# paulsengroup/modle

Hardware: AMD Instinct MI355X
Metric: simulated cells/sec (whole node), GRCh38 default barriers (higher is better)
Workload: dtype u32/f64

## Files before the change

modle_amd/csrc/sim_cell.h:

```cpp
#pragma once
#include "sim_rng.h"

namespace modle_dev {

struct Cell {
  const Params* p;
  const Interval* iv;
  Workspace ws;
  WaveLds lds;
  Rng g;
  u32 n_lefs;
  u32 n_active;
  u32 hist_len;
  u32 hist_head;
  u32 error;
  u32 n_hit[2];
  u32 n_rel;
  bool rel_valid;
  u32 n_bound;
  u32 n_keys;
  bool keys_valid;
  u32 n_disp[2];
  bool disp_valid;
  u32 max_fwd_move;
  bool inv_valid[2];
  bool filter_on;
  bool by_id_valid;
  u32 pair_seq;
  u32 pair_interval;
  bool pair_on;
  bool ring_lent;
#ifdef MODLE_PHASE_TIMERS
  u64 ph[16];
#endif
};
#if defined(MODLE_SUBTIMER_LEFBAR) || defined(MODLE_SUBTIMER_STATS) || defined(MODLE_SUBTIMER_RANK)
#define MODLE_SUBTIMER 1
#endif
#ifdef MODLE_SUBTIMER
#define MODLE_PH_ACTIVATION 1
#else
#define MODLE_PH_ACTIVATION 14
#endif
#ifdef MODLE_PHASE_TIMERS
#define PHASE(c, i, ...)                          \
  do {                                            \
    const u64 ph_t0_ = wave::clock();             \
    __VA_ARGS__;                                  \
    (c).ph[i] += wave::clock() - ph_t0_;          \
  } while (0)
#else
#define PHASE(c, i, ...) \
  do {                   \
    __VA_ARGS__;         \
  } while (0)
#endif
constexpr u32 REL_CAP = 2 * SORT_LDS_CAP;
constexpr u32 RANK_KEY_CAP = SORT_LDS_CAP - 1;
constexpr u32 RANK_KEY_CAP_BIG = RNG_RING - 1;
constexpr u32 RING_SPILL_AT = 64;
constexpr u32 ERR_LIST_OVERFLOW = 1;
constexpr u32 ERR_TRIAL_OVERFLOW = 2;
constexpr u32 ERR_INTERNAL = 3;
constexpr u32 ERR_MOVE_RANGE = 5;
constexpr bool NARROW_MOVES = sizeof(move_t) < sizeof(u32);

MODLE_DEV Interval interval_in_device_memory(const Interval& iv) {
  Interval g = iv;
  g.bar_pos = wave::as_global(iv.bar_pos);
  g.bar_dir = wave::as_global(iv.bar_dir);
  g.bar_stp_active = wave::as_global(iv.bar_stp_active);
  g.bar_stp_inactive = wave::as_global(iv.bar_stp_inactive);
  g.bar_occupancy = wave::as_global(iv.bar_occupancy);
  g.contacts = wave::as_global(iv.contacts);
  g.occupancy_1d = wave::as_global(iv.occupancy_1d);
  g.missed_updates = wave::as_global(iv.missed_updates);
  g.bar_bucket = wave::as_global(iv.bar_bucket);
  return g;
}

template <class T>
MODLE_DEV void swap_ptr(T*& a, T*& b) {
  T* t = a;
  a = b;
  b = t;
}

template <class T>
MODLE_DEV void swap_with_scratch(T*& a, u32*& scratch) {
  T* t = a;
  a = reinterpret_cast<T*>(scratch);
  scratch = reinterpret_cast<u32*>(t);
}
MODLE_DEV lefid_t* as_ids(u32* scratch) { return reinterpret_cast<lefid_t*>(scratch); }
MODLE_DEV const lefid_t* as_ids(const u32* scratch) { return reinterpret_cast<const lefid_t*>(scratch); }
MODLE_DEV move_t* as_moves(u32* scratch) { return reinterpret_cast<move_t*>(scratch); }
MODLE_DEV const move_t* as_moves(const u32* scratch) { return reinterpret_cast<const move_t*>(scratch); }

MODLE_DEV u32 bar_lower_bound(const Interval& iv, u64 key) {
  const u32 nb = iv.n_barriers;
  if (key <= iv.start) return 0;
  const u64 b = (key - iv.start) >> iv.bucket_shift;
  if (b >= iv.n_buckets) return nb;
  u32 i = iv.bar_bucket[b];
  while (i < nb && iv.bar_pos[i] < key) ++i;
  return i;
}

MODLE_DEV u32 lower_bound_u32(const u32* a, u32 n, u32 key) {
  u32 lo = 0, hi = n;
  while (lo < hi) {
    const u32 mid = (lo + hi) >> 1;
    if (a[mid] < key) lo = mid + 1; else hi = mid;
  }
  return lo;
}

template <bool FWD>
MODLE_DEV_NOINLINE void ensure_inverse(Cell& c) {
  if (c.inv_valid[FWD ? 1 : 0]) return;
  Workspace& ws = c.ws;
  const u32 n = wave::uniform(c.n_active);
  const u32 lane = wave::lane();
  const lefid_t* ids = FWD ? ws.f_id : ws.r_id;
  u32* rank = FWD ? ws.f_rank : ws.r_rank;
  const u32 nblk = (n + 255) / 256;
  for (u32 t = 0; t < nblk; ++t) {
    const u32 w = 256 * t + 4 * lane;
    const wave::U32x4 I = wave::ld4(ids, w < n ? w : 0u);
#pragma unroll
    for (u32 q = 0; q < 4; ++q) {
      if (w + q < n) rank[I.v[q]] = w + q;
    }
  }
  wave::sync_mem();
  c.inv_valid[FWD ? 1 : 0] = true;
}
MODLE_DEV void ensure_inverse_both(Cell& c) {
  ensure_inverse<false>(c);
  ensure_inverse<true>(c);
}

constexpr u32 RANK_HARD = 0x80000000u;
constexpr u32 RANK_FILTER_WORDS = SORT_LDS_CAP;
constexpr u32 RANK_FILTER_BITS = 64 * RANK_FILTER_WORDS;
MODLE_DEV void rank_filter_clear(Cell& c, u32 n_ids) {
  u64* bm = c.lds.sort_lds;
  const u32 nw = umin(RANK_FILTER_WORDS, (n_ids + 63) / 64);
  wave::lockstep();
  for (u32 k = wave::lane(); k < nw; k += 64) bm[k] = 0;
  wave::sync_lds();
}
MODLE_DEV void rank_filter_add_mask(Cell& c, u32 first, u64 members) {
  u64* bm = c.lds.sort_lds;
  if (wave::lane() == 0) bm[(first / 64) % RANK_FILTER_WORDS] |= members;
}
MODLE_DEV void rank_filter_add_id(Cell& c, u32 id) {
  u32* bm = reinterpret_cast<u32*>(c.lds.sort_lds);
  wave::lds_or_u32(&bm[(id % RANK_FILTER_BITS) >> 5], 1u << (id & 31u));
}
MODLE_DEV bool rank_filter_test(const Cell& c, u32 id) {
  const u32* bm = reinterpret_cast<const u32*>(c.lds.sort_lds);
  return ((bm[(id % RANK_FILTER_BITS) >> 5] >> (id & 31u)) & 1u) != 0;
}

}
```

modle_amd/csrc/sim_collisions.h:

```cpp
#pragma once

namespace modle_dev {

struct BoundaryCounts {
  u32 n5, n3;
};

MODLE_DEV_NOINLINE BoundaryCounts detect_boundaries(Cell& c) {
  Workspace& ws = c.ws;
  const u32 n = wave::uniform(c.n_active);
  const u32 lane = wave::lane();
  const u32 start = c.iv->start, last = c.iv->end - 1;
  const u32 first_fwd_pos = ws.f_pos[0];
  u32 last_rev_pos = 0;
  for (u32 top = n; top > 0;) {
    const u32 cnt = umin(64u, top);
    const bool act = lane < cnt;
    const u32 P = wave::ld_sel(ws.r_pos, top - 1 - lane, act, UNBOUND);
    const u64 m = wave::ballot(act && P != UNBOUND);
    if (m != 0) {
      last_rev_pos = wave::bcast(P, static_cast<u32>(wave::ctz64(m)));
      break;
    }
    top -= cnt;
// ... 805 lines not shown
        const u32 ps = wave_prefix_sum_u32(lane_cnt);
        const u32 first = n_listed + ps - lane_cnt;
#pragma unroll
        for (u32 j = 0; j < 4; ++j) {
          if (has[j]) {
            unit_rank[first + before[j]] = k[j];
            unit_entry[first + before[j]] = entry[j];
            unit_key[first + before[j]] = FWD ? hi_key[j] : lo_key[j];
          }
        }
        n_listed += wave::bcast(ps, 63);
      }
    }
  }
  wave::sync_mem();
  return n_listed;
}

template <bool FWD>
MODLE_DEV_NOINLINE void resolve_listed_units(Cell& c, u32 n_listed) {
  Workspace& ws = c.ws;
  const Params& p = *c.p;
  const u32 lane = wave::lane();
  const u32 nh = wave::uniform(c.n_hit[FWD ? 1 : 0]);
  const u32* hpos = ws.hit_pos[FWD ? 1 : 0];
  const u32* hidx = ws.hit_idx[FWD ? 1 : 0];
  const u32* unit_rank = ws.tmp[0];
  const u32* unit_entry = ws.tmp[1];
  const u32* unit_key = ws.tmp[2];
  u32* coll = FWD ? ws.f_coll : ws.r_coll;
  u32* barpos = stalling_barrier_positions<FWD>(ws);
  const f64 pb_major = wave::own_regs(p.pblock_major), pb_minor = wave::own_regs(p.pblock_minor);
  const bool major_trial = pb_major != 1.0, minor_trial = pb_minor != 1.0;
  const auto visit = [&](u32 e_lo, u32 e_hi, u32 q) { return FWD ? e_hi - 1 - q : e_lo + q; };
  for (u32 base = 0; base < n_listed; base += 64) {
    const u32 u = base + lane;
    const bool act = u < n_listed;
    const u32 k = wave::ld_sel(unit_rank, u, act, 0u);
    const u32 e0 = wave::ld_sel(unit_entry, u, act, 0u);
    const u32 key = wave::ld_sel(unit_key, u, act, 0u);
    u32 e_lo = e0, e_hi = e0;
    if (act) {
      if (!FWD) {
        while (e_lo > 0 && hpos[e_lo - 1] >= key) --e_lo;
      } else {
        while (e_hi < nh && hpos[e_hi] < key) ++e_hi;
      }
    }
    u32 ntr = 0;
    for (u32 q = 0; q < e_hi - e_lo; ++q) {
      const bool is_major = (hidx[visit(e_lo, e_hi, q)] & HITBAR_HARD) != 0;
      ntr += (is_major ? major_trial : minor_trial) ? 1u : 0u;
    }
    u32 off = wave_prefix_sum_u32(ntr);
    const u32 total = wave::bcast(off, 63);
    off -= ntr;
    const auto pick = [&](u32 first, u32& w_entry) {
      u32 t = 0;
      w_entry = 0xFFFFFFFFu;
      for (u32 q = 0; q < e_hi - e_lo; ++q) {
        const u32 e = visit(e_lo, e_hi, q);
        const bool is_major = (hidx[e] & HITBAR_HARD) != 0;
        bool hit = true;
        if (is_major ? major_trial : minor_trial) {
          hit = bernoulli_raw(rng_peek(c.g, c.g.pos + first + t), is_major ? pb_major : pb_minor);
          ++t;
        }
        if (hit) w_entry = e;
      }
    };
#ifdef MODLE_EMU_TRACE_RANK
    if (lane == 0) fprintf(stderr, "lef_bar_trials: %s batch of %u units, %u trials%s\n", FWD ? "fwd" : "rev",
                           umin(64u, n_listed - base), total, total > RNG_BLOCK ? " (resolved in rounds)" : "");
#endif
    u32 w_entry = 0xFFFFFFFFu;
    if (total <= RNG_BLOCK) {
      if (total != 0) rng_ensure(c.g, total);
      if (act) pick(off, w_entry);
      rng_advance(c.g, total);
    } else {
      u64 pend = wave::ballot(act);
      u32 base_tr = 0;
      while (pend != 0) {
        const bool mine_pending = ((pend >> lane) & 1u) != 0;
        const bool fits = mine_pending && (off + ntr - base_tr <= RNG_BLOCK);
        const u64 fm = wave::ballot(fits);
        if (fm == 0) {
          const u32 l = static_cast<u32>(wave::ctz64(pend));
          const u32 lo = wave::bcast(e_lo, l), hi = wave::bcast(e_hi, l);
          u32 w = 0xFFFFFFFFu;
          for (u32 q = 0; q < hi - lo; ++q) {
            const u32 e = FWD ? hi - 1 - q : lo + q;
            const bool is_major = (wave::uniform(hidx[e]) & HITBAR_HARD) != 0;
            bool hit = true;
            if (is_major ? major_trial : minor_trial) hit = bernoulli_raw(rng_next(c.g), is_major ? pb_major : pb_minor);
            if (hit) w = e;
          }
          if (lane == l) w_entry = w;
          base_tr += wave::bcast(ntr, l);
          pend &= ~(u64(1) << l);
        } else {
          const u32 l_last_fit = static_cast<u32>(63 - wave::clz64(fm));
          const u32 cnt = wave::bcast(off + ntr, l_last_fit) - base_tr;
          if (cnt != 0) rng_ensure(c.g, cnt);
          if (fits) pick(off - base_tr, w_entry);
          rng_advance(c.g, cnt);
          base_tr += cnt;
          pend &= ~fm;
        }
      }
    }
    if (w_entry != 0xFFFFFFFFu) {
      const u32 wd = hidx[w_entry];
      coll[k] = cw_make(wd & ~HITBAR_HARD, EV_COLLISION | EV_LEF_BAR) | ((wd & HITBAR_HARD) ? CW_HARD : 0u);
      barpos[k] = hpos[w_entry];
    }
  }
  wave::sync_mem();
}

template <bool FWD>
MODLE_DEV_NOINLINE void detect_lef_bar(Cell& c, BoundaryCounts bc) {
  if (wave::uniform(c.iv->n_barriers) == 0) return;
  if (!lef_bar_trials_needed(*c.p)) {
    detect_lef_bar_det<FWD>(c, bc);
    return;
  }
  const u32 n_listed = detect_lef_bar_sweep<FWD, true>(c, bc);
  if (n_listed != 0) resolve_listed_units<FWD>(c, n_listed);
}

MODLE_DEV void lef_lef_collision_pos(u32 rev_p, u32 fwd_p, u32 rev_move, u32 fwd_move,
                                     u32& out_rev, u32& out_fwd) {
  const f64 relative_speed = static_cast<f64>(rev_move) + static_cast<f64>(fwd_move);
  const f64 ttc = static_cast<f64>(rev_p - fwd_p) / relative_speed;
  const u32 cpos = fwd_p + static_cast<u32>(wave::f_round(static_cast<f64>(fwd_move) * ttc));
  if (cpos == fwd_p) {
    out_rev = cpos + 1;
    out_fwd = cpos;
  } else {
    out_rev = cpos;
    out_fwd = cpos - 1;
  }
}

MODLE_DEV u32 stalling_barrier_pos(const Interval& iv, u32 word) {
  const u32 idx = cw_index(word);
  return idx < iv.n_barriers ? iv.bar_pos[idx] : 0u;
}

#ifndef MODLE_PRIMARY_BACK
#define MODLE_PRIMARY_BACK 128
#endif
constexpr u32 PRIMARY_BACK = MODLE_PRIMARY_BACK;
static_assert(PRIMARY_BACK + 128 <= STAGE_CAP, "the slice must reach the block's last rank");
struct PrimaryBatch {
  wave::U32x2 R, rev_move;
  u32 sp[STAGE_CAP / 64];
};
template <class Op>
MODLE_DEV void primary_load_batch(Op op, const Workspace& ws, u32 n, u32 base, u32 w0, u32 lane,
                                  PrimaryBatch& b, bool rev_side) {
  if (rev_side) {
    const u32 k0 = base + 2 * lane;
    const u32 kq = k0 < n ? k0 : 0u;
    b.R = wave::ld2(ws.r_pos, kq);
    b.rev_move = wave::ld2(ws.r_move, kq);
  }
#pragma unroll
  for (u32 q = 0; q < STAGE_CAP / 64; ++q) {
    const u32 t = lane + 64 * q;
    b.sp[q] = op(ws.f_pos, w0 + t, w0 + t < n, UNBOUND, b.sp[q]);
  }
}

MODLE_DEV_NOINLINE void detect_primary(Cell& c, BoundaryCounts bc, bool fuse_correct) {
  Workspace& ws = c.ws;
  const Params& p = *c.p;
  const Interval& iv = *c.iv;
  const u32 n = wave::uniform(c.n_active);
  if (bc.n5 == n || bc.n3 == n) return;
  const u32 lane = wave::lane();
  const u32 i2 = bc.n3 == 0 ? n : n - (bc.n3 - 1);
  const f64 p_collide = 1.0 - p.p_bypass;
  const bool never_collide = p.p_bypass != 0.0 && p_collide == 0.0;
  const bool trials = p.p_bypass != 0.0 && !never_collide;
  const u32 prim = EV_COLLISION | EV_LEF_LEF_PRIMARY;
  u32* stage = c.lds.stage;
  u32* const q_k = ws.tmp[0];
  u32* const q_pf = ws.tmp[1];
  u32* const dump = reinterpret_cast<u32*>(ws.sort_keys) + 2 * lane;
  const u64 fwd_reach = wave::uniform(c.max_fwd_move);
  u32 n_cand = 0;
  u32 carry_pos = 0;
  const u32 first = bc.n5;
  const auto slice_start = [](u32 base) { return base > PRIMARY_BACK ? base - PRIMARY_BACK : 0u; };
  {
    const u32 b0 = first & ~1u;
    PrimaryBatch pa, pb;
    primary_load_batch(wave::LdRaw{}, ws, n, b0, slice_start(b0), lane, pa, true);
    if (b0 + 128 < n) primary_load_batch(wave::LdRaw{}, ws, n, b0 + 128, slice_start(b0 + 128), lane, pb, true);
    const auto block = [&](PrimaryBatch& cur, u32 base) {
      const u32 w0 = slice_start(base);
      primary_load_batch(wave::LdMask{}, ws, n, base, w0, lane, cur, false);
      u32 k[2], R[2], rev_move[2];
      bool act[2];
#pragma unroll
      for (u32 j = 0; j < 2; ++j) {
        k[j] = base + 2 * lane + j;
        act[j] = k[j] >= first && k[j] < n;
        R[j] = act[j] ? cur.R.v[j] : UNBOUND;
        rev_move[j] = act[j] ? cur.rev_move.v[j] : 0u;
      }
      wave::lockstep();
#pragma unroll
      for (u32 q = 0; q < STAGE_CAP / 64; ++q) stage[lane + 64 * q] = cur.sp[q];
      wave::sync_lds();
      if (base + 256 < n) primary_load_batch(wave::LdRaw{}, ws, n, base + 256, slice_start(base + 256), lane, cur, true);
      const u32 prev_in = wave::shfl_up1(R[1]);
      const u32 Rprev0 = lane > 0 ? prev_in : carry_pos;
      u32 lo[2] = {0, 0};
      static_assert(STAGE_CAP == 256, "the search below covers 256 entries");
#pragma unroll
      for (u32 sft = 128; sft >= 1; sft >>= 1) {
        u32 sv[2];
#pragma unroll
        for (u32 j = 0; j < 2; ++j) sv[j] = stage[lo[j] + sft - 1];
        wave::sched_fence();
#pragma unroll
        for (u32 j = 0; j < 2; ++j) {
          if (sv[j] < R[j]) lo[j] += sft;
        }
        wave::sched_fence();
      }
      const u32 st_last = stage[STAGE_CAP - 1];
      u32 pf[2] = {0, 0};
      bool beyond = false;
#pragma unroll
      for (u32 j = 0; j < 2; ++j) {
        u32 l = lo[j];
        if (l == STAGE_CAP - 1 && st_last < R[j]) l = STAGE_CAP;
        pf[j] = umin(w0 + l, n);
        beyond = beyond || (act[j] && ((l == 0 && w0 > 0) || (l == STAGE_CAP && w0 + STAGE_CAP < n)));
      }
      if (wave::any(beyond)) {
#pragma unroll
        for (u32 j = 0; j < 2; ++j) {
          const u32 l = pf[j] - w0;
          if (act[j] && ((l == 0 && w0 > 0) || (l == STAGE_CAP && w0 + STAGE_CAP < n)))
            pf[j] = lower_bound_u32(ws.f_pos, n, R[j]);
          wave::pin(pf[j]);
        }
      }
      u32 F[2];
      bool has[2], staged[2];
#pragma unroll
      for (u32 j = 0; j < 2; ++j) {
        has[j] = act[j] && pf[j] >= 1 && pf[j] < i2;
        const u32 kf = pf[j] - 1;
        staged[j] = has[j] && kf >= w0 && kf - w0 < STAGE_CAP;
        F[j] = stage[staged[j] ? kf - w0 : 0u];
      }
      wave::sched_fence();
      if (wave::any((has[0] && !staged[0]) || (has[1] && !staged[1]))) {
#pragma unroll
        for (u32 j = 0; j < 2; ++j) {
          if (has[j] && !staged[j]) F[j] = ws.f_pos[pf[j] - 1];
          wave::pin(F[j]);
        }
      }
      bool cand[2];
#pragma unroll
      for (u32 j = 0; j < 2; ++j) {
        const u32 Rprev = j == 0 ? Rprev0 : R[0];
        const bool first_after = (k[j] == first) || Rprev <= F[j];
        const u32 delta = R[j] - F[j];
        cand[j] = has[j] && first_after && static_cast<u64>(delta) < static_cast<u64>(rev_move[j]) + fwd_reach;
      }
      const u64 cm0 = wave::ballot(cand[0]), cm1 = wave::ballot(cand[1]);
      {
        const u64 lt = lanemask_lt(lane);
        const u32 e0 = n_cand + static_cast<u32>(wave::popc64(cm0 & lt) + wave::popc64(cm1 & lt));
        const u32 e1 = e0 + (cand[0] ? 1u : 0u);
        *(cand[0] ? &q_k[e0] : dump) = k[0];
        *(cand[0] ? &q_pf[e0] : dump + 1) = pf[0];
        *(cand[1] ? &q_k[e1] : dump) = k[1];
        *(cand[1] ? &q_pf[e1] : dump + 1) = pf[1];
      }
      n_cand += static_cast<u32>(wave::popc64(cm0) + wave::popc64(cm1));
      carry_pos = wave::bcast(R[1], 63);
    };
    for (u32 base = b0; base < n; base += 256) {
      block(pa, base);
      if (base + 128 < n) block(pb, base + 128);
    }
  }
  wave::sync_mem();
  struct PairRegs {
    u32 k, pf, R, rev_move, rev_id, rc, rbp, F, fwd_move, fwd_id, fc, fbp;
  };
  const auto load_pairs = [&](u32 base, u32 kk, u32 pp, PairRegs& r) {
    const bool in = base + lane < n_cand;
    const u32 k = in ? kk : 0u, kf = in ? pp - 1 : 0u;
    r.k = kk;
    r.pf = pp;
    r.R = wave::LdRaw{}(ws.r_pos, k, true, 0, 0u);
    r.rev_move = wave::LdRaw{}(ws.r_move, k, true, 0, 0u);
    r.rev_id = wave::LdRaw{}(ws.r_id, k, true, 0, 0u);
    r.rc = wave::LdRaw{}(ws.r_coll, k, true, 0, 0u);
    r.rbp = wave::LdRaw{}(stalling_barrier_positions<false>(ws), k, true, 0, 0u);
    r.F = wave::LdRaw{}(ws.f_pos, kf, true, 0, 0u);
    r.fwd_move = wave::LdRaw{}(ws.f_move, kf, true, 0, 0u);
    r.fwd_id = wave::LdRaw{}(ws.f_id, kf, true, 0, 0u);
    r.fc = wave::LdRaw{}(ws.f_coll, kf, true, 0, 0u);
    r.fbp = wave::LdRaw{}(stalling_barrier_positions<true>(ws), kf, true, 0, 0u);
  };
  const auto list_k = [&](u32 base) { return wave::ld_sel(q_k, base + lane, base + lane < n_cand, 0u); };
  const auto list_pf = [&](u32 base) { return wave::ld_sel(q_pf, base + lane, base + lane < n_cand, 1u); };
  PairRegs pcur;
  u32 nk = 0, np = 1;
  if (n_cand != 0) {
    load_pairs(0, list_k(0), list_pf(0), pcur);
    if (64 < n_cand) {
      nk = list_k(64);
      np = list_pf(64);
    }
  }
  for (u32 base = 0; base < n_cand; base += 64) {
    const PairRegs q = pcur;
    if (base + 64 < n_cand) {
      load_pairs(base + 64, nk, np, pcur);
      if (base + 128 < n_cand) {
        nk = list_k(base + 128);
        np = list_pf(base + 128);
      }
    }
    const bool valid = base + lane < n_cand;
    const u32 delta = q.R - q.F;
    const bool cand = valid && static_cast<u64>(delta) < static_cast<u64>(q.rev_move) + q.fwd_move;
    const u64 cm = wave::ballot(cand);
    bool hit = cand && !never_collide;
    if (trials && cm != 0) {
      const u32 cnt = static_cast<u32>(wave::popc64(cm));
      rng_ensure(c.g, cnt);
      const u32 t = static_cast<u32>(wave::popc64(cm & lanemask_lt(lane)));
      hit = cand && bernoulli_raw(rng_peek(c.g, c.g.pos + t), p_collide);
      rng_advance(c.g, cnt);
    }
    const auto handle_hit = [&](u32 pf_h, u32 k_h, u32 R_h, u32 F_h, u32 rev_move_h, u32 fwd_move_h, u32 rev_id_k_h,
                                u32 fwd_id_s_h, u32 rc_k_h, u32 fc_s_h, u32 rbp_k_h, u32 fbp_s_h) {
      const u32 kf = pf_h - 1;
      const u32 rev_id = rev_id_k_h, fwd_id = fwd_id_s_h;
      u32 cpos_rev, cpos_fwd;
      lef_lef_collision_pos(R_h, F_h, rev_move_h, fwd_move_h, cpos_rev, cpos_fwd);
      const u32 rc = rc_k_h, fc = fc_s_h;
      const bool rev_occ = cw_occurred(rc), fwd_occ = cw_occurred(fc);
      u32 rev_other = 0, fwd_other = 0;
      const bool rev_odd = rev_occ && !cw_occurred_as(rc, EV_LEF_BAR);
      const bool fwd_odd = fwd_occ && !cw_occurred_as(fc, EV_LEF_BAR);
      if (rev_odd || fwd_odd) {
        if (rev_odd) rev_other = stalling_barrier_pos(iv, rc);
        if (fwd_odd) fwd_other = stalling_barrier_pos(iv, fc);
        wave::pin(rev_other);
        wave::pin(fwd_other);
      }
      bool both = false;
      if (!rev_occ && !fwd_occ) {
        ws.r_coll[k_h] = cw_make(fwd_id, prim);
        ws.f_coll[kf] = cw_make(rev_id, prim);
        both = true;
      } else if (rev_occ && !fwd_occ) {
        const u32 barrier_pos = rev_odd ? rev_other : rbp_k_h;
        ws.f_coll[kf] = cw_make(rev_id, prim);
        if (cpos_fwd > barrier_pos) {
          ws.r_coll[k_h] = cw_make(fwd_id, prim);
          both = true;
        } else if (fuse_correct && cw_occurred_as(rc, EV_LEF_BAR)) {
          const u32 rev_move_stalled = (R_h - barrier_pos) - 1;
          ws.f_move[kf] = (R_h - rev_move_stalled) - F_h - 1;
        }
      } else if (!rev_occ && fwd_occ) {
        const u32 barrier_pos = fwd_odd ? fwd_other : fbp_s_h;
        ws.r_coll[k_h] = cw_make(fwd_id, prim);
        if (cpos_rev < barrier_pos) {
          ws.f_coll[kf] = cw_make(rev_id, prim);
          both = true;
        } else if (fuse_correct && cw_occurred_as(fc, EV_LEF_BAR)) {
          const u32 fwd_move_stalled = (barrier_pos - F_h) - 1;
          ws.r_move[k_h] = R_h - (F_h + fwd_move_stalled) - 1;
        }
      }
      if (both && fuse_correct) {
        ws.r_move[k_h] = R_h - cpos_rev;
        ws.f_move[kf] = cpos_fwd - F_h;
      }
    };
    if (wave::any(hit)) {
      if (hit) handle_hit(q.pf, q.k, q.R, q.F, q.rev_move, q.fwd_move, q.rev_id, q.fwd_id, q.rc, q.fc, q.rbp, q.fbp);
    }
  }
  wave::sync_mem();
}

MODLE_DEV_NOINLINE void correct_moves_primary_standalone(Cell& c) {
  ensure_inverse_both(c);
  Workspace& ws = c.ws;
  const u32 n = wave::uniform(c.n_active);
  const u32 lane = wave::lane();
  for (u32 base = 0; base < n; base += 64) {
    const u32 k = base + lane;
    if (k < n) {
      const u32 rc = ws.r_coll[k];
      if (cw_occurred_as(rc, EV_LEF_LEF_PRIMARY)) {
        const u32 kf = ws.f_rank[cw_index(rc)];
        const u32 fc = ws.f_coll[kf];
        if (cw_occurred_as(fc, EV_LEF_LEF_PRIMARY)) {
          u32 p1, p2;
          lef_lef_collision_pos(ws.r_pos[k], ws.f_pos[kf], ws.r_move[k], ws.f_move[kf], p1, p2);
          ws.r_move[k] = ws.r_pos[k] - p1;
          ws.f_move[kf] = p2 - ws.f_pos[kf];
        } else if (cw_occurred_as(fc, EV_LEF_BAR)) {
          ws.r_move[k] = ws.r_pos[k] - (ws.f_pos[kf] + ws.f_move[kf]) - 1;
        }
      }
    }
  }
  wave::sync_mem();
  for (u32 base = 0; base < n; base += 64) {
    const u32 k = base + lane;
    if (k < n) {
      const u32 fc = ws.f_coll[k];
      if (cw_occurred_as(fc, EV_LEF_LEF_PRIMARY)) {
        const u32 kr = ws.r_rank[cw_index(fc)];
        if (cw_occurred_as(ws.r_coll[kr], EV_LEF_BAR))
          ws.f_move[k] = (ws.r_pos[kr] - ws.r_move[kr]) - ws.f_pos[k] - 1;
      }
    }
  }
  wave::sync_mem();
}

constexpr u32 SEC_CONT = 0x40000000u;
constexpr u32 SEC_BOCC = 0x80000000u;

MODLE_DEV u32 sec_compose(u32 earlier, u32 later) {
  const u32 p = (later & 1u) | ((later >> 1) & earlier & 1u);
  const u32 q = (later >> 1) & (earlier >> 1) & 1u;
  return p | (q << 1);
}
MODLE_DEV u32 wave_prefix_sec_compose(u32 v) {
#define MODLE_STEP(S) v = sec_compose(wave::scan_move<S>(v, 2u), v);
  MODLE_SCAN_STEPS(MODLE_STEP)
#undef MODLE_STEP
  return v;
}

template <bool FWD>
struct SecondaryFilter {
  struct Blk {
    wave::U32x4 P, M, C, B;
  };
  const u32 *pos, *coll, *barpos;
  move_t *moves, *dump_m;
  u32 *q_k, *dump;
  u32 n, lane, nblk, cap, n_cand, carry_pos, carry_coll;
  i32 f_first;
  bool correct_lef_bar, do_secondary, carry_pending;
  Blk cur;

  MODLE_DEV_MEMBER u32 word0(u32 t) const { return (FWD ? nblk - 1 - t : t) * 256 + 4 * (FWD ? 63 - lane : lane); }
  MODLE_DEV_MEMBER void load_blk(u32 t, Blk& r) const {
    const u32 w = word0(t);
    const u32 wq = w < n ? w : 0u;
    r.P = wave::ld4(pos, wq);
    r.M = wave::ld4(moves, wq);
    r.C = wave::ld4(coll, wq);
    r.B = wave::ld4(barpos, wq);
  }
  MODLE_DEV_MEMBER void init(Cell& c, BoundaryCounts bc, u32 list_cap, bool lef_bar, bool secondary) {
    Workspace& ws = c.ws;
    n = wave::uniform(c.n_active);
    lane = wave::lane();
    pos = FWD ? ws.f_pos : ws.r_pos;
    coll = FWD ? ws.f_coll : ws.r_coll;
    barpos = stalling_barrier_positions<FWD>(ws);
    moves = FWD ? ws.f_move : ws.r_move;
    q_k = FWD ? ws.tmp[1] : ws.tmp[0];
    dump = reinterpret_cast<u32*>(ws.sort_keys) + 2 * lane + (FWD ? 1 : 0);
    dump_m = reinterpret_cast<move_t*>(dump);
    cap = list_cap;
    correct_lef_bar = lef_bar;
    do_secondary = secondary;
    f_first = FWD ? static_cast<i32>(bc.n3 == 0 ? n - 1 : n - bc.n3) - 1
                  : static_cast<i32>(umax(1u, bc.n5));
    nblk = (n + 255) / 256;
    n_cand = 0;
    carry_pos = 0;
    carry_coll = 0;
    carry_pending = false;
    load_blk(0, cur);
  }
  MODLE_DEV_MEMBER void step(u32 t) {
    const Blk g = cur;
    if (t + 1 < nblk) load_blk(t + 1, cur);
    const u32 w = word0(t);
    u32 k[4], P[4], M[4], C[4];
    bool act[4];
#pragma unroll
    for (u32 j = 0; j < 4; ++j) {
      const u32 q = FWD ? 3 - j : j;
      k[j] = w + q;
      act[j] = k[j] < n;
      P[j] = act[j] ? g.P.v[q] : 0u;
      C[j] = act[j] ? g.C.v[q] : 0u;
      const u32 M0 = g.M.v[q];
      M[j] = M0;
      if (correct_lef_bar && act[j] && cw_occurred_as(C[j], EV_LEF_BAR)) {
        const u32 bp = g.B.v[q];
        M[j] = (FWD ? bp - P[j] : P[j] - bp) - 1;
      }
      *((act[j] && M[j] != M0) ? &moves[k[j]] : dump_m) = static_cast<move_t>(M[j]);
    }
    const u32 pP_in = wave::shfl_up1(P[3]), pC_in = wave::shfl_up1(C[3]);
    bool pot[4], bocc[4];
    u32 fn = 2u;
#pragma unroll
    for (u32 j = 0; j < 4; ++j) {
      const u32 bP = j == 0 ? (lane > 0 ? pP_in : carry_pos) : P[j - 1];
      const u32 bC = j == 0 ? (lane > 0 ? pC_in : carry_coll) : C[j - 1];
      const i32 kk = static_cast<i32>(k[j]);
      const bool follower = do_secondary && act[j] && (FWD ? (kk <= f_first) : (kk >= f_first));
      pot[j] = follower && !cw_occurred(C[j]) &&
               (FWD ? static_cast<u64>(P[j]) + M[j] >= bP : static_cast<u64>(P[j]) - M[j] <= bP);
      bocc[j] = cw_occurred(bC);
      fn = sec_compose(fn, (pot[j] && bocc[j] ? 1u : 0u) | (pot[j] ? 2u : 0u));
    }
    const u32 incl = wave_prefix_sec_compose(fn);
    const u32 before_in = wave::shfl_up1(incl);
    const u32 before = lane > 0 ? before_in : 2u;
    bool x_prev = ((before & 1u) | ((before >> 1) & (carry_pending ? 1u : 0u))) != 0;
    bool x[4], cont[4];
    u32 lane_cnt = 0;
#pragma unroll
    for (u32 j = 0; j < 4; ++j) {
      cont[j] = x_prev;
      x[j] = pot[j] && (bocc[j] || x_prev);
      x_prev = x[j];
      lane_cnt += x[j] ? 1u : 0u;
    }
    const u32 ps = wave_prefix_sum_u32(lane_cnt);
    u32 e = n_cand + ps - lane_cnt;
#pragma unroll
    for (u32 j = 0; j < 4; ++j) {
      *((x[j] && e < cap) ? &q_k[e] : dump) = k[j] | (cont[j] ? SEC_CONT : 0u) | (bocc[j] ? SEC_BOCC : 0u);
// ... 461 lines not shown
```

modle_amd/csrc/sim_epoch.h:

```cpp
#pragma once

namespace modle_dev {

MODLE_DEV_NOINLINE void reset_cell_buffers(Cell& c) {
  Workspace& ws = c.ws;
  const u32 L = wave::uniform(c.n_lefs);
  const u32 lane = wave::lane();
  for (u32 base = 0; base < L; base += 64) {
    const u32 i = base + lane;
    if (i < L) {
      ws.r_pos[i] = UNBOUND;
      ws.f_pos[i] = UNBOUND;
      ws.epoch[i] = UNBOUND;
      ws.r_id[i] = i;
      ws.f_id[i] = i;
      ws.r_rank[i] = i;
      ws.f_rank[i] = i;
      ws.r_move[i] = 0;
      ws.f_move[i] = 0;
      ws.r_coll[i] = 0;
      ws.f_coll[i] = 0;
      ws.stall[i] = 0;
    }
  }
// ... 66 lines not shown
  u64 s[4] = {0, 0, 0, 0};
  for (u32 base = 0; base < c.n_active; base += 64) {
    const u32 k = base + lane;
    if (k < c.n_active) {
      const u64 w = k + 1;
      s[0] += w * c.ws.r_pos[k] + c.ws.r_id[k];
      s[1] += w * c.ws.f_pos[k] + c.ws.f_id[k];
      s[2] += w * c.ws.r_move[k];
      s[3] += w * c.ws.f_move[k];
    }
  }
#pragma unroll
  for (u32 q = 0; q < 4; ++q) {
#pragma unroll
    for (u32 d = 1; d < 64; d <<= 1) {
      const u64 o = wave::shfl_down(s[q], d);
      if (lane + d < 64) s[q] += o;
    }
  }
  if (lane == 0) {
    u64* rec = tr + (epoch * TRACE_STAGES + stage) * TRACE_WORDS_PER_STAGE;
    rec[0] = c.g.pos;
    rec[1] = s[0];
    rec[2] = s[1];
    rec[3] = s[2];
    rec[4] = s[3];
    rec[5] = (static_cast<u64>(c.n_active) << 32) | (stage + 1);
  }
}
#endif

#ifdef MODLE_STATE_LOG
MODLE_DEV_NOINLINE void log_internal_state(Cell& c, u64 epoch, bool burnin) {
  u64* log = c.lds.state_log;
  if (log == nullptr || epoch >= c.lds.state_log_cap) return;
  Workspace& ws = c.ws;
  const u32 n = wave::uniform(c.n_active);
  const u32 lane = wave::lane();
  u32* flag = ws.tmp[2];
  u32 st_rev = 0, st_fwd = 0, st_both = 0, n_bar = 0, n_prim = 0, n_sec = 0;
  u64 part = 0;
  for (u32 base = 0; base < n; base += 64) {
    const u32 k = base + lane;
    const bool act = k < n;
    const u32 rc = wave::ld_sel(ws.r_coll, k, act, 0);
    const u32 P = wave::ld_sel(ws.r_pos, k, act, UNBOUND);
    if (act) flag[ws.r_id[k]] = cw_occurred(rc) ? 1u : 0u;
    st_rev += static_cast<u32>(wave::popc64(wave::ballot(act && cw_occurred(rc))));
    n_bar += static_cast<u32>(wave::popc64(wave::ballot(act && cw_occurred_as(rc, EV_LEF_BAR))));
    n_prim += static_cast<u32>(wave::popc64(wave::ballot(act && cw_occurred_as(rc, EV_LEF_LEF_PRIMARY))));
    n_sec += static_cast<u32>(wave::popc64(wave::ballot(act && cw_occurred_as(rc, EV_LEF_LEF_SECONDARY))));
    if (act && P != UNBOUND) part -= static_cast<u64>(P - ws.r_move[k]);
  }
  wave::sync_mem();
  for (u32 base = 0; base < n; base += 64) {
    const u32 k = base + lane;
    const bool act = k < n;
    const u32 fc = wave::ld_sel(ws.f_coll, k, act, 0);
    const u32 P = wave::ld_sel(ws.f_pos, k, act, UNBOUND);
    const bool both = act && cw_occurred(fc) && flag[ws.f_id[k]] != 0;
    st_fwd += static_cast<u32>(wave::popc64(wave::ballot(act && cw_occurred(fc))));
    st_both += static_cast<u32>(wave::popc64(wave::ballot(both)));
    n_bar += static_cast<u32>(wave::popc64(wave::ballot(act && cw_occurred_as(fc, EV_LEF_BAR))));
    n_prim += static_cast<u32>(wave::popc64(wave::ballot(act && cw_occurred_as(fc, EV_LEF_LEF_PRIMARY))));
    n_sec += static_cast<u32>(wave::popc64(wave::ballot(act && cw_occurred_as(fc, EV_LEF_LEF_SECONDARY))));
    if (act && P != UNBOUND) part += static_cast<u64>(P + ws.f_move[k]);
  }
#pragma unroll
  for (u32 sft = 1; sft < 64; sft <<= 1) {
    const u64 o = wave::shfl_down(part, sft);
    if (lane + sft < 64) part += o;
  }
  const u64 loop_sum = wave::bcast(part, 0);
  u32 n_occ = 0;
  const u32 nb = wave::uniform(c.iv->n_barriers);
  for (u32 base = 0; base < nb; base += 64) {
    const u32 i = base + lane;
    n_occ += static_cast<u32>(wave::popc64(wave::ballot(i < nb && ws.bar_active[i] != 0)));
  }
  if (lane == 0) {
    u64* rec = log + epoch * STATE_LOG_WORDS;
    rec[0] = epoch | (burnin ? (u64(1) << 63) : 0);
    rec[1] = n_occ;
    rec[2] = n;
    rec[3] = st_rev;
    rec[4] = st_fwd;
    rec[5] = st_both;
    rec[6] = n_bar;
    rec[7] = n_prim;
    rec[8] = n_sec;
    rec[9] = loop_sum;
  }
  wave::sync_mem();
}
#else
MODLE_DEV void log_internal_state(Cell&, u64, bool) {}
#endif

MODLE_DEV u32 simulate_cell(const Params& p, const Interval& iv, const Task& task,
                            const Workspace& ws, const WaveLds& lds, CellResult& res) {
  Cell c;
#ifdef MODLE_PHASE_TIMERS
  const u64 t_cell = wave::clock();
#endif
  const Interval ivg = interval_in_device_memory(iv);
  init_cell(c, p, ivg, ws, lds, task.num_lefs, task.prng);
  c.pair_interval = task.interval;
  reset_cell_buffers(c);

  u64 epoch = 0, num_burnin_epochs = 0, num_contacts = 0;
  u64 sum_active = 0, events_done = 0, sim_epochs = 0;
  bool burnin_completed = false;
  u32 status = 0;
  const f64 lef_binding_rate_burnin =
      static_cast<f64>(task.num_lefs) / static_cast<f64>(p.burnin_target_epochs_for_lef_activation);

  barriers_init_states(c);
  c.rel_valid = true;
  if (p.skip_burnin) {
    activate_lefs(c, 0, c.n_lefs);
    burnin_completed = true;
  }
  for (;; ++epoch) {
    if (p.target_contact_density >= 0) {
      if (num_contacts >= task.num_target_contacts) break;
    } else if (epoch - num_burnin_epochs >= task.num_target_epochs) {
      break;
    }
    if (lds.abort_flag != nullptr && (epoch & 15u) == 0 &&
        wave::uniform(wave::load_system_u32(lds.abort_flag)) != 0) {
      status = ERR_CANCELLED;
      break;
    }
    bool stats_due = false;
    c.by_id_valid = false;
    if (!burnin_completed) {
      do {
        ++num_burnin_epochs;
        if (c.n_active != c.n_lefs) {
          PHASE(c, MODLE_PH_ACTIVATION, const u64 k = poisson_exact(c.g, lef_binding_rate_burnin);
                const u64 na = static_cast<u64>(c.n_active) + k;
                activate_lefs(c, c.n_active, na < c.n_lefs ? static_cast<u32>(na) : c.n_lefs));
        } else {
          stats_due = true;
        }
      } while (c.n_active == 0);
    }
    PHASE(c, 1, if (c.rel_valid) phase_bind_listed(c, static_cast<u32>(epoch));
          else {
            phase_bind(c, static_cast<u32>(epoch));
            c.n_bound = c.n_active;
          });
    if (stats_due) {
      PHASE(c, 0, compute_loop_size_stats(c); burnin_completed = evaluate_burnin(c));
      burnin_completed = burnin_completed && epoch > p.min_burnin_epochs;
      if (!burnin_completed && epoch >= p.max_burnin_epochs) {
        burnin_completed = true;
        activate_lefs(c, c.n_active, c.n_lefs);
      }
    }
    trace_stage(c, epoch, 0);
    c.pair_on = pair_helper_present(lds);
    const bool offload = c.pair_on && !burnin_completed;
    if (offload) pair_request(c, burnin_completed, task.interval);
    PHASE(c, 2, rank_update<false>(c, false));
    PHASE(c, 3, rank_update<true>(c, false));
    trace_stage(c, epoch, 1);
    if (c.error != 0) {
      const u32 first_error = c.error;
      if (offload) (void)pair_take_back(c);
      status = first_error;
      break;
    }

    if (burnin_completed) {
      PHASE(c, 4, num_contacts += phase_sample_contacts(c, task.contacts_per_epoch,
                                                        task.num_target_contacts, num_contacts,
                                                        events_done));
      trace_stage(c, epoch, 5);
      if (task.num_target_contacts != 0 && num_contacts >= task.num_target_contacts) break;
    }

    sum_active += c.n_active;
    ++sim_epochs;
    if (offload) {
      c.max_fwd_move = 0xFFFFFFFFu;
      bool handed = false;
      PHASE(c, 5, handed = pair_wait(c, PAIR_MOVES));
      if (!handed) {
        status = c.error;
        break;
      }
      phase_adjust_moves_by_id(c);
      trace_stage(c, epoch, 2);
      PHASE(c, 7, handed = pair_take_back(c));
      if (!handed) {
        status = c.error;
        break;
      }
    } else {
      phase_generate_moves(c, burnin_completed);
      trace_stage(c, epoch, 2);
      PHASE(c, 7, barriers_next_state(c));
    }
    if (NARROW_MOVES && c.error != 0) {
      status = c.error;
      break;
    }
    const bool coll_ok = phase_process_collisions(c);
    trace_stage(c, epoch, 3);
    if (!coll_ok) {
      status = c.error;
      break;
    }
    log_internal_state(c, epoch, !burnin_completed);
    PHASE(c, 13, phase_extrude_and_release(c, burnin_completed));
    trace_stage(c, epoch, 4);
  }

  trace_stage(c, epoch, 6);
#ifdef MODLE_PHASE_TIMERS
#ifndef MODLE_SUBTIMER
  c.ph[15] = wave::clock() - t_cell;
#endif
#ifdef MODLE_PROF_RNG
  c.ph[14] = c.g.gen_ticks;
#endif
  if (lds.phase_ticks != nullptr && wave::lane() == 0) {
    for (int i = 0; i < 16; ++i) wave::atomic_add_u64(lds.phase_ticks + i, c.ph[i]);
  }
  wave::lockstep();
#endif
  res.epochs = epoch;
  res.burnin_epochs = num_burnin_epochs;
  res.num_contacts = num_contacts;
  res.raws_consumed = c.g.pos;
  rng_final_state(c.g, res.prng_final);
  res.sum_active_lefs = sum_active;
  res.sampling_events = events_done;
  res.sim_epochs = sim_epochs;
  return status;
}

}
```

Measured before the change: 368.2.

## Search primary collision partners near rank with short bisection over LDS slice

Rewrites the first pass of detect_primary to process 256 ranks per iteration with four ranks per lane. The forward-position slice now lives in the LDS sort buffer, and the full 8-step binary search is replaced by a short search in a window just below each rank. A longer slice search or a device-memory lower_bound runs only when the partner falls below that window. Lookup depth drops from eight to four steps for the common case, at the cost of a larger register footprint and an added fallback path. Optional subtimers and counters are added behind compile flags.

Result: faster. 373.8, median of 6 (+1.5%).

```diff
diff --git a/modle_amd/csrc/sim_cell.h b/modle_amd/csrc/sim_cell.h
--- a/modle_amd/csrc/sim_cell.h
+++ b/modle_amd/csrc/sim_cell.h
@@ -34,8 +34,13 @@
   u64 ph[16];
 #endif
 };
-#if defined(MODLE_SUBTIMER_LEFBAR) || defined(MODLE_SUBTIMER_STATS) || defined(MODLE_SUBTIMER_RANK)
+#if defined(MODLE_SUBTIMER_LEFBAR) || defined(MODLE_SUBTIMER_STATS) || defined(MODLE_SUBTIMER_RANK) || \
+    defined(MODLE_SUBTIMER_PRIMARY) || defined(MODLE_SUBTIMER_BURNIN) || defined(MODLE_COUNT_PRIMARY_FAR)
 #define MODLE_SUBTIMER 1
+#endif
+#if defined(MODLE_SUBTIMER_LEFBAR) + defined(MODLE_SUBTIMER_STATS) + defined(MODLE_SUBTIMER_RANK) + defined(MODLE_SUBTIMER_PRIMARY) + \
+        defined(MODLE_SUBTIMER_BURNIN) + defined(MODLE_COUNT_PRIMARY_FAR) > 1
+#error "one measurement inside a phase per build: they share slots 14 and 15"
 #endif
 #ifdef MODLE_SUBTIMER
 #define MODLE_PH_ACTIVATION 1
diff --git a/modle_amd/csrc/sim_collisions.h b/modle_amd/csrc/sim_collisions.h
--- a/modle_amd/csrc/sim_collisions.h
+++ b/modle_amd/csrc/sim_collisions.h
@@ -981,27 +981,19 @@
 #ifndef MODLE_PRIMARY_BACK
 #define MODLE_PRIMARY_BACK 128
 #endif
+#ifndef MODLE_PRIMARY_NEAR
+#define MODLE_PRIMARY_NEAR 16
+#endif
 constexpr u32 PRIMARY_BACK = MODLE_PRIMARY_BACK;
-static_assert(PRIMARY_BACK + 128 <= STAGE_CAP, "the slice must reach the block's last rank");
-struct PrimaryBatch {
-  wave::U32x2 R, rev_move;
-  u32 sp[STAGE_CAP / 64];
+constexpr u32 PRIMARY_NEAR = MODLE_PRIMARY_NEAR;
+constexpr u32 PRIMARY_SLICE_Q = (PRIMARY_BACK + 256 + 63) / 64;
+static_assert(64 * PRIMARY_SLICE_Q <= 2 * SORT_LDS_CAP, "the slice must fit the LDS sort buffer");
+static_assert(PRIMARY_NEAR >= 2 && (PRIMARY_NEAR & (PRIMARY_NEAR - 1)) == 0 && PRIMARY_NEAR <= 256,
+              "the short search halves its step down to one");
+struct PrimaryBlk {
+  wave::U32x4 R, rev_move;
+  u32 sp[PRIMARY_SLICE_Q];
 };
-template <class Op>
-MODLE_DEV void primary_load_batch(Op op, const Workspace& ws, u32 n, u32 base, u32 w0, u32 lane,
-                                  PrimaryBatch& b, bool rev_side) {
-  if (rev_side) {
-    const u32 k0 = base + 2 * lane;
-    const u32 kq = k0 < n ? k0 : 0u;
-    b.R = wave::ld2(ws.r_pos, kq);
-    b.rev_move = wave::ld2(ws.r_move, kq);
-  }
-#pragma unroll
-  for (u32 q = 0; q < STAGE_CAP / 64; ++q) {
-    const u32 t = lane + 64 * q;
-    b.sp[q] = op(ws.f_pos, w0 + t, w0 + t < n, UNBOUND, b.sp[q]);
-  }
-}
 
 MODLE_DEV_NOINLINE void detect_primary(Cell& c, BoundaryCounts bc, bool fuse_correct) {
   Workspace& ws = c.ws;
@@ -1015,7 +1007,6 @@
   const bool never_collide = p.p_bypass != 0.0 && p_collide == 0.0;
   const bool trials = p.p_bypass != 0.0 && !never_collide;
   const u32 prim = EV_COLLISION | EV_LEF_LEF_PRIMARY;
-  u32* stage = c.lds.stage;
   u32* const q_k = ws.tmp[0];
   u32* const q_pf = ws.tmp[1];
   u32* const dump = reinterpret_cast<u32*>(ws.sort_keys) + 2 * lane;
@@ -1024,107 +1015,141 @@
   u32 carry_pos = 0;
   const u32 first = bc.n5;
   const auto slice_start = [](u32 base) { return base > PRIMARY_BACK ? base - PRIMARY_BACK : 0u; };
+#ifdef MODLE_SUBTIMER_PRIMARY
+  const u64 t_pass1 = wave::clock();
+#endif
   {
-    const u32 b0 = first & ~1u;
-    PrimaryBatch pa, pb;
-    primary_load_batch(wave::LdRaw{}, ws, n, b0, slice_start(b0), lane, pa, true);
-    if (b0 + 128 < n) primary_load_batch(wave::LdRaw{}, ws, n, b0 + 128, slice_start(b0 + 128), lane, pb, true);
-    const auto block = [&](PrimaryBatch& cur, u32 base) {
+    u32* const sl = reinterpret_cast<u32*>(c.lds.sort_lds);
+    const auto load_blk = [&](u32 base, PrimaryBlk& r) {
+      const u32 w = base + 4 * lane;
+      const u32 wq = w < n ? w : 0u;
+      r.R = wave::ld4(ws.r_pos, wq);
+      r.rev_move = wave::ld4(ws.r_move, wq);
+      const u32 t0 = slice_start(base) + lane;
+#pragma unroll
+      for (u32 q = 0; q < PRIMARY_SLICE_Q; ++q) r.sp[q] = wave::LdRaw{}(ws.f_pos, umin(t0 + 64 * q, n - 1), true, 0, 0u);
+    };
+    PrimaryBlk cur;
+    load_blk(first & ~255u, cur);
+    for (u32 base = first & ~255u; base < n; base += 256) {
+      const PrimaryBlk g = cur;
       const u32 w0 = slice_start(base);
-      primary_load_batch(wave::LdMask{}, ws, n, base, w0, lane, cur, false);
-      u32 k[2], R[2], rev_move[2];
-      bool act[2];
-#pragma unroll
-      for (u32 j = 0; j < 2; ++j) {
-        k[j] = base + 2 * lane + j;
-        act[j] = k[j] >= first && k[j] < n;
-        R[j] = act[j] ? cur.R.v[j] : UNBOUND;
-        rev_move[j] = act[j] ? cur.rev_move.v[j] : 0u;
-      }
       wave::lockstep();
 #pragma unroll
-      for (u32 q = 0; q < STAGE_CAP / 64; ++q) stage[lane + 64 * q] = cur.sp[q];
+      for (u32 q = 0; q < PRIMARY_SLICE_Q; ++q) sl[lane + 64 * q] = g.sp[q];
       wave::sync_lds();
-      if (base + 256 < n) primary_load_batch(wave::LdRaw{}, ws, n, base + 256, slice_start(base + 256), lane, cur, true);
-      const u32 prev_in = wave::shfl_up1(R[1]);
+      if (base + 256 < n) load_blk(base + 256, cur);
+      const u32 k0 = base + 4 * lane;
+      u32 R[4], rev_move[4];
+      bool act[4];
+#pragma unroll
+      for (u32 j = 0; j < 4; ++j) {
+        act[j] = k0 + j >= first && k0 + j < n;
+        R[j] = act[j] ? g.R.v[j] : UNBOUND;
+        rev_move[j] = act[j] ? g.rev_move.v[j] : 0u;
+      }
+      const u32 prev_in = wave::shfl_up1(R[3]);
       const u32 Rprev0 = lane > 0 ? prev_in : carry_pos;
-      u32 lo[2] = {0, 0};
-      static_assert(STAGE_CAP == 256, "the search below covers 256 entries");
-#pragma unroll
-      for (u32 sft = 128; sft >= 1; sft >>= 1) {
-        u32 sv[2];
-#pragma unroll
-        for (u32 j = 0; j < 2; ++j) sv[j] = stage[lo[j] + sft - 1];
+      const u32 a0 = k0 - w0;
+      u32 es[4], lo[4];
+#pragma unroll
+      for (u32 j = 0; j < 4; ++j) {
+        es[j] = umax(a0 + j, PRIMARY_NEAR) - PRIMARY_NEAR;
+        lo[j] = es[j] + 1;
+      }
+#pragma unroll
+      for (u32 sft = PRIMARY_NEAR / 2; sft >= 1; sft >>= 1) {
+        u32 sv[4];
+#pragma unroll
+        for (u32 j = 0; j < 4; ++j) sv[j] = sl[lo[j] + sft - 1];
         wave::sched_fence();
 #pragma unroll
-        for (u32 j = 0; j < 2; ++j) {
+        for (u32 j = 0; j < 4; ++j) {
           if (sv[j] < R[j]) lo[j] += sft;
         }
         wave::sched_fence();
       }
-      const u32 st_last = stage[STAGE_CAP - 1];
-      u32 pf[2] = {0, 0};
-      bool beyond = false;
-#pragma unroll
-      for (u32 j = 0; j < 2; ++j) {
-        u32 l = lo[j];
-        if (l == STAGE_CAP - 1 && st_last < R[j]) l = STAGE_CAP;
-        pf[j] = umin(w0 + l, n);
-        beyond = beyond || (act[j] && ((l == 0 && w0 > 0) || (l == STAGE_CAP && w0 + STAGE_CAP < n)));
-      }
-      if (wave::any(beyond)) {
-#pragma unroll
-        for (u32 j = 0; j < 2; ++j) {
-          const u32 l = pf[j] - w0;
-          if (act[j] && ((l == 0 && w0 > 0) || (l == STAGE_CAP && w0 + STAGE_CAP < n)))
-            pf[j] = lower_bound_u32(ws.f_pos, n, R[j]);
+      u32 pf[4], F[4];
+      bool below[4];
+      bool far = false;
+#pragma unroll
+      for (u32 j = 0; j < 4; ++j) F[j] = sl[lo[j] - 1];
+      wave::sched_fence();
+#pragma unroll
+      for (u32 j = 0; j < 4; ++j) {
+        const bool edge = lo[j] == es[j] + 1 && F[j] >= R[j];
+        pf[j] = w0 + lo[j] - (edge ? 1u : 0u);
+        below[j] = act[j] && edge && (es[j] != 0 || w0 != 0);
+        far = far || below[j];
+      }
+#ifdef MODLE_COUNT_PRIMARY_FAR
+      u32 n_dev = 0;
+#pragma unroll
+      for (u32 j = 0; j < 4; ++j) c.ph[14] += static_cast<u32>(wave::popc64(wave::ballot(below[j])));
+#endif
+      if (wave::any(far)) {
+#pragma unroll
+        for (u32 j = 0; j < 4; ++j) {
+          if (below[j]) {
+            u32 l = 0, h = es[j];
+            while (l < h) {
+              const u32 mid = (l + h) >> 1;
+              if (sl[mid] < R[j]) l = mid + 1;
+              else h = mid;
+            }
+            pf[j] = w0 + l;
+            if (l != 0) {
+              F[j] = sl[l - 1];
+            } else if (w0 > 0) {
+              pf[j] = lower_bound_u32(ws.f_pos, n, R[j]);
+              if (pf[j] >= 1) F[j] = ws.f_pos[pf[j] - 1];
+#ifdef MODLE_COUNT_PRIMARY_FAR
+              n_dev |= 1u << j;
+#endif
+#ifdef MODLE_EMU_TRACE_PRIMARY
+              fprintf(stderr, "detect_primary: rank %u device memory\n", k0 + j);
+#endif
+            }
+#ifdef MODLE_EMU_TRACE_PRIMARY
+            fprintf(stderr, "detect_primary: rank %u rest of the slice\n", k0 + j);
+#endif
+          }
           wave::pin(pf[j]);
-        }
-      }
-      u32 F[2];
-      bool has[2], staged[2];
-#pragma unroll
-      for (u32 j = 0; j < 2; ++j) {
-        has[j] = act[j] && pf[j] >= 1 && pf[j] < i2;
-        const u32 kf = pf[j] - 1;
-        staged[j] = has[j] && kf >= w0 && kf - w0 < STAGE_CAP;
-        F[j] = stage[staged[j] ? kf - w0 : 0u];
-      }
-      wave::sched_fence();
-      if (wave::any((has[0] && !staged[0]) || (has[1] && !staged[1]))) {
-#pragma unroll
-        for (u32 j = 0; j < 2; ++j) {
-          if (has[j] && !staged[j]) F[j] = ws.f_pos[pf[j] - 1];
           wave::pin(F[j]);
         }
-      }
-      bool cand[2];
-#pragma unroll
-      for (u32 j = 0; j < 2; ++j) {
-        const u32 Rprev = j == 0 ? Rprev0 : R[0];
-        const bool first_after = (k[j] == first) || Rprev <= F[j];
+#ifdef MODLE_COUNT_PRIMARY_FAR
+#pragma unroll
+        for (u32 j = 0; j < 4; ++j) c.ph[15] += static_cast<u32>(wave::popc64(wave::ballot(((n_dev >> j) & 1u) != 0)));
+#endif
+      }
+      bool cand[4];
+      u32 lane_cnt = 0;
+#pragma unroll
+      for (u32 j = 0; j < 4; ++j) {
+        const bool has = act[j] && pf[j] >= 1 && pf[j] < i2;
+        const u32 Rprev = j == 0 ? Rprev0 : R[j - 1];
+        const bool first_after = (k0 + j == first) || Rprev <= F[j];
         const u32 delta = R[j] - F[j];
-        cand[j] = has[j] && first_after && static_cast<u64>(delta) < static_cast<u64>(rev_move[j]) + fwd_reach;
-      }
-      const u64 cm0 = wave::ballot(cand[0]), cm1 = wave::ballot(cand[1]);
-      {
-        const u64 lt = lanemask_lt(lane);
-        const u32 e0 = n_cand + static_cast<u32>(wave::popc64(cm0 & lt) + wave::popc64(cm1 & lt));
-        const u32 e1 = e0 + (cand[0] ? 1u : 0u);
-        *(cand[0] ? &q_k[e0] : dump) = k[0];
-        *(cand[0] ? &q_pf[e0] : dump + 1) = pf[0];
-        *(cand[1] ? &q_k[e1] : dump) = k[1];
-        *(cand[1] ? &q_pf[e1] : dump + 1) = pf[1];
-      }
-      n_cand += static_cast<u32>(wave::popc64(cm0) + wave::popc64(cm1));
-      carry_pos = wave::bcast(R[1], 63);
-    };
-    for (u32 base = b0; base < n; base += 256) {
-      block(pa, base);
-      if (base + 128 < n) block(pb, base + 128);
+        cand[j] = has && first_after && static_cast<u64>(delta) < static_cast<u64>(rev_move[j]) + fwd_reach;
+        lane_cnt += cand[j] ? 1u : 0u;
+      }
+      const u32 ps = wave_prefix_sum_u32(lane_cnt);
+      u32 e = n_cand + ps - lane_cnt;
+#pragma unroll
+      for (u32 j = 0; j < 4; ++j) {
+        *(cand[j] ? &q_k[e] : dump) = k0 + j;
+        *(cand[j] ? &q_pf[e] : dump + 1) = pf[j];
+        e += cand[j] ? 1u : 0u;
+      }
+      n_cand += wave::bcast(ps, 63);
+      carry_pos = wave::bcast(R[3], 63);
     }
   }
   wave::sync_mem();
+#ifdef MODLE_SUBTIMER_PRIMARY
+  const u64 t_pass2 = wave::clock();
+  c.ph[14] += t_pass2 - t_pass1;
+#endif
   struct PairRegs {
     u32 k, pf, R, rev_move, rev_id, rc, rbp, F, fwd_move, fwd_id, fc, fbp;
   };
@@ -1229,6 +1254,9 @@
     }
   }
   wave::sync_mem();
+#ifdef MODLE_SUBTIMER_PRIMARY
+  c.ph[15] += wave::clock() - t_pass2;
+#endif
 }
 
 MODLE_DEV_NOINLINE void correct_moves_primary_standalone(Cell& c) {
diff --git a/modle_amd/csrc/sim_epoch.h b/modle_amd/csrc/sim_epoch.h
--- a/modle_amd/csrc/sim_epoch.h
+++ b/modle_amd/csrc/sim_epoch.h
@@ -242,7 +242,11 @@
             c.n_bound = c.n_active;
           });
     if (stats_due) {
+#ifdef MODLE_SUBTIMER_BURNIN
+      PHASE(c, 0, PHASE(c, 14, compute_loop_size_stats(c)); PHASE(c, 15, burnin_completed = evaluate_burnin(c)));
+#else
       PHASE(c, 0, compute_loop_size_stats(c); burnin_completed = evaluate_burnin(c));
+#endif
       burnin_completed = burnin_completed && epoch > p.min_burnin_epochs;
       if (!burnin_completed && epoch >= p.max_burnin_epochs) {
         burnin_completed = true;
```
